# mihaidusmanu/local-feature-refinement

Measured on AMD Instinct MI355X. Metric: edges_per_s, higher is better.
Workload: dtype f64; 1 GPU; config4: synthetic match graph, 1344 images, 147000 tracks/GPU (mean length 6), 5001070 directed edges/GPU, Gaussian flows, seed 2+rank; edges_per_gpu=5001070, tracks_per_gpu=147000, components_per_gpu=147000, parallelism=components sharded, 1 rank(s), no data-path collective

## Files before the change

local-feature-refinement_amd/csrc/lfr_batch.hip:

```cpp
#include <hip/hip_runtime.h>

#include <algorithm>
#include <atomic>
#include <array>
#include <chrono>
#include <memory>
#include <string>
#include <thread>
#include <cstdio>
#include <cstdlib>
#include <cstring>
#include <vector>

#include "lfr_assemble.hpp"
#include "lfr_batch.hpp"
#include "lfr_internal.hpp"

using lfr::CompDesc;
using lfr::CompInfoDev;
using lfr::EdgeRec;
using lfr::KernelArgs;
using lfr::PackedRanges;
using lfr::block_lds_bytes;
using lfr::ensure_mirrors;
// ... 502 lines not shown
    return LFR_OK;
}

int lfr_hip_trim(int device) {
    lfr::DevCtx *ctx = lfr::dev_ctx(device);
    if (!ctx) return LFR_ERR_HIP;
    ctx->trim();
    return LFR_OK;
}

void lfr_batch_free(lfr_batch *b) { delete b; }

int lfr_batch_create(const lfr_problem *ph, int device, int shard_rank, int shard_world, int tukey_variant,
                     lfr_batch **out) {
    if (!ph || !out || shard_world < 1 || shard_rank < 0 || shard_rank >= shard_world ||
        (tukey_variant != LFR_TUKEY_CERES1 && tukey_variant != LFR_TUKEY_CERES2)) {
        lfr::set_error("bad argument"); return LFR_ERR_ARG;
    }
    *out = nullptr;
    const lfr::Problem &p = ph->p;
    lfr::DevCtx *ctx = lfr::dev_ctx(device);
    if (!ctx) return LFR_ERR_HIP;
    HIP_TRY(hipSetDevice(device));
    std::unique_ptr<lfr_batch> b(new lfr_batch());
    b->device = device; b->ctx = ctx; b->tukey_variant = tukey_variant; b->shard_world = shard_world;
    { const char *e = getenv("LFR_SERIAL_CLASSES"); b->serial = e && e[0] == '1'; }
    b->n_graph_nodes = p.g->n_nodes();
    b->graph = p.g; b->n_graph_matches = p.g->n_matches();
    int rc = p.host_batch ? create_from_host(b.get(), p, shard_rank, shard_world) : create_on_device(b.get(), p, shard_rank, shard_world);
    if (rc != LFR_OK) return rc;
    if ((rc = finish_workspace(b.get(), p)) != LFR_OK) return rc;
    host_trace("lfr_batch_create: workspace done");
    if (!(b->ev_fork = ctx->event_acquire(false))) return LFR_ERR_HIP;
    if (b->class_begin[lfr::KC_COUNT] > b->class_begin[lfr::KC_BLOCK]) {
        if (!(b->side_stream = ctx->side_stream(0))) return LFR_ERR_HIP;
        for (int cls = lfr::KC_BLOCK; cls < lfr::KC_COUNT; ++cls)
            if (b->class_begin[cls + 1] > b->class_begin[cls] && !(b->wg_stream[cls] = ctx->side_stream(1 + cls))) return LFR_ERR_HIP;
        {
            const int wg_begin = b->class_begin[lfr::KC_BLOCK], n_wg = b->class_begin[lfr::KC_COUNT] - wg_begin;
            hipStream_t so = ctx->s_main;
            size_t tmp_bytes = 0;
            HIP_TRY(rocprim::radix_sort_pairs<LfrRadixSortConfig>(nullptr, tmp_bytes, (const uint32_t *)nullptr, (uint32_t *)nullptr, (const uint32_t *)nullptr,
                                                                   (uint32_t *)nullptr, (size_t)n_wg, 0u, 27u, so));
            if (!b->order_slab.init(ctx, 16 * (size_t)n_wg + tmp_bytes + 4096)) return LFR_ERR_NOMEM;
            b->d_wg_order = b->order_slab.take_n<uint32_t>(n_wg);
            uint32_t *keys = b->order_slab.take_n<uint32_t>(n_wg), *keys_sorted = b->order_slab.take_n<uint32_t>(n_wg), *vals = b->order_slab.take_n<uint32_t>(n_wg);
            void *tmp = b->order_slab.take(tmp_bytes);
            if (!b->d_wg_order || !keys || !keys_sorted || !vals || !tmp) { lfr::set_error("order slab exhausted"); return LFR_ERR_NOMEM; }
            hipLaunchKernelGGL(k_wg_order_keys, dim3((n_wg + 255) / 256), dim3(256), 0, so, b->d_descs + wg_begin, n_wg,
                               b->class_begin[lfr::KC_BLOCK_M] - wg_begin, b->class_begin[lfr::KC_BLOCK_L] - wg_begin, b->class_begin[lfr::KC_GLOBAL] - wg_begin,
                               keys, vals, wg_begin);
            HIP_TRY(hipGetLastError());
            HIP_TRY(rocprim::radix_sort_pairs<LfrRadixSortConfig>(tmp, tmp_bytes, keys, keys_sorted, vals, b->d_wg_order, (size_t)n_wg, 0u, 27u, so));
            if (!(b->ev_order = ctx->event_acquire(false))) return LFR_ERR_HIP;
            HIP_TRY(hipEventRecord(b->ev_order, so));
        }
        host_trace("lfr_batch_create: hand-out order enqueued");
        const int lds_s = (int)block_lds_bytes(std::max(b->class_max_rows[lfr::KC_BLOCK], 2));
        const int lds_m = (int)block_lds_bytes(std::max(b->class_max_rows[lfr::KC_BLOCK_M], 2));
        const int lds_l = (int)block_lds_bytes(std::max(b->class_max_rows[lfr::KC_BLOCK_L], 2));
        if ((rc = lfr::reserve_block_lds(lds_s, lds_m, lds_l)) != LFR_OK) return rc;
    }
    {
        int64_t best = -1;
        for (int cls = 0; cls < lfr::KC_BLOCK; ++cls) if (b->class_edges[cls] > best) { best = b->class_edges[cls]; b->packed_slot = cls; }
    }
// ... 74 lines not shown
        HIP_TRY(hipGetLastError());
        return LFR_OK;
    };
    const bool have_side = b->class_begin[lfr::KC_COUNT] > b->class_begin[lfr::KC_BLOCK];
    if (b->serial) {
        for (int cls = 0; cls < lfr::KC_COUNT; ++cls) {
            a.desc_begin = b->class_begin[cls]; a.desc_end = b->class_begin[cls + 1]; a.cls = cls;
            const int n = a.desc_end - a.desc_begin;
            if (n <= 0) continue;
            recorded |= 1u << cls;
            HIP_TRY(hipEventRecord(b->ev[2 + 2 * cls], st));
            {
                const int grid = (n + kCompsPerBlock[cls] - 1) / kCompsPerBlock[cls];
                if (cls < lfr::KC_BLOCK) lfr::launch_group_class(cls, a, b->fused, grid, st);
                else { const int rc = launch_block(cls, st); if (rc != LFR_OK) return rc; }
                HIP_TRY(hipGetLastError());
            }
            HIP_TRY(hipEventRecord(b->ev[3 + 2 * cls], st));
        }
    } else {
        PackedRanges r;
        int nb = 0;
        for (int i = 0; i < 5; ++i) {
            const int cls = kPackedOrder[i];
            r.blk_begin[i] = nb;
            r.desc_begin[i] = b->class_begin[cls]; r.desc_end[i] = b->class_begin[cls + 1];
            const int n = r.desc_end[i] - r.desc_begin[i];
            nb += (n + kCompsPerBlock[cls] - 1) / kCompsPerBlock[cls];
        }
        r.blk_begin[5] = nb;
        const bool alias = !have_side && !materialised;
        auto launch_packed = [&](hipStream_t cs) -> int {
            if (!alias) HIP_TRY(hipEventRecord(b->ev[2 + 2 * b->packed_slot], cs));
            lfr::launch_packed(a, r, b->fused, nb, cs);
            HIP_TRY(hipGetLastError());
            if (!alias) HIP_TRY(hipEventRecord(b->ev[3 + 2 * b->packed_slot], cs));
            recorded |= 1u << b->packed_slot;
            if (alias) recorded |= kPackedEventsAliased;
            return LFR_OK;
        };
        auto launch_big = [&](int cls, hipStream_t cs) -> int {
            HIP_TRY(hipEventRecord(b->ev[2 + 2 * cls], cs));
            const int rc = launch_block(cls, cs);
            if (rc != LFR_OK) return rc;
            HIP_TRY(hipEventRecord(b->ev[3 + 2 * cls], cs));
            recorded |= 1u << cls;
            return LFR_OK;
        };
        if (!have_side) {
            if (nb > 0) { const int rc = launch_packed(st); if (rc != LFR_OK) return rc; }
        } else {
            static const std::array<int, 4> kBigOrder = [] {
                std::array<int, 4> o = {lfr::KC_GLOBAL, lfr::KC_BLOCK_M, lfr::KC_BLOCK_L, lfr::KC_BLOCK};
                if (const char *e = getenv("LFR_WG_ORDER")) {
                    int v[4];
                    if (sscanf(e, "%d,%d,%d,%d", &v[0], &v[1], &v[2], &v[3]) == 4) {
                        unsigned seen = 0;
                        for (int i = 0; i < 4; ++i) if (v[i] >= lfr::KC_BLOCK && v[i] < lfr::KC_COUNT) seen |= 1u << v[i];
                        if (seen == (0xfu << lfr::KC_BLOCK)) for (int i = 0; i < 4; ++i) o[i] = v[i];
                    }
                }
                return o;
            }();
            int first = -1, n_big = 0;
            for (int i = 0; i < 4; ++i) if (b->class_begin[kBigOrder[i] + 1] > b->class_begin[kBigOrder[i]]) { if (first < 0) first = kBigOrder[i]; ++n_big; }
            if (n_big > 1 || nb > 0) HIP_TRY(hipEventRecord(b->ev_fork, st));
            { const int rc = launch_big(first, st); if (rc != LFR_OK) return rc; }
            for (int i = 0; i < 4; ++i) {
// ... 470 lines not shown
```

local-feature-refinement_amd/csrc/lfr_batch.hpp:

```cpp
#pragma once

#include <hip/hip_runtime.h>

#include <cstdint>
#include <memory>
#include <vector>

#include "lfr_internal.hpp"

#define HIP_TRY(expr)                                                                         \
    do {                                                                                      \
        hipError_t _e = (expr);                                                               \
        if (_e != hipSuccess) {                                                               \
            lfr::set_error("%s failed: %s", #expr, hipGetErrorString(_e));                    \
            return LFR_ERR_HIP;                                                               \
        }                                                                                     \
    } while (0)

namespace lfr {

struct CompInfoDev {
    int32_t iterations, termination, n_successful, n_ls_evals, n_cand_evals, exec_passes;
    double final_cost;
};
// ... 82 lines not shown
    unsigned int *d_team_ctl = nullptr;
    double *d_team_red = nullptr;
    uint32_t team_work[3] = {0xffffffffu, 0xffffffffu, 0xffffffffu};
    int team_wgs = 0;
    uint32_t team_patience_us = 50000u;
    std::vector<int64_t> tree_comp_stats;
    int64_t tree_tiles = 0, tree_dense_tiles = 0;
    uint64_t *d_ws_off = nullptr, *d_es_off = nullptr;
    bool fused = false;
    uint32_t packed_edges = 0;
    uint32_t *d_edge_ref = nullptr, *d_edge_word = nullptr;
    std::shared_ptr<lfr::DevProblem> dev_hold;
    unsigned long long *d_prof = nullptr;
    lfr::NodeInc *d_node_inc = nullptr;
    uint32_t *d_in_idx = nullptr;
    uint32_t *d_desc_component = nullptr, *d_desc_class = nullptr, *d_desc_tracks = nullptr;
    bool mirrors_valid = false;
    std::vector<lfr::CompDesc> descs;
    std::vector<int64_t> desc_component;
    std::vector<int32_t> desc_class, desc_tracks;
    std::vector<uint32_t> node_ids;
    double *h_positions = nullptr;
    size_t h_positions_bytes = 0;
    float *h_positions_f32 = nullptr, *d_positions_f32 = nullptr;
    size_t h_positions_f32_bytes = 0, d_positions_f32_bytes = 0;
    static constexpr int kSlots = 64;
    static constexpr int kEvPerSlot = 2 * (lfr::KC_COUNT + 1);
    hipEvent_t ev_ring[kSlots * kEvPerSlot];
    hipEvent_t *ev = ev_ring;
    uint32_t ev_recorded[kSlots] = {};
    int64_t n_solves = 0;
    bool serial = false;
    hipEvent_t ev_fork = nullptr;
    lfr::DevArena order_slab;
    uint32_t *d_wg_order = nullptr;
    hipEvent_t ev_order = nullptr;
    hipStream_t side_stream = nullptr;
    hipStream_t wg_stream[lfr::KC_COUNT] = {nullptr};
    hipStream_t last_stream = nullptr;
    int packed_slot = 0;
    double h2d_ms = 0.0;
    std::vector<lfr::CompInfoDev> infos;
    bool infos_valid = false;
    const lfr::Graph *graph = nullptr;
    int64_t n_graph_matches = 0;
    BwdState *bwd = nullptr;
    CovState *cov = nullptr;

    lfr_batch() { for (auto &e : ev_ring) e = nullptr; }
    ~lfr_batch() {
        bwd_free(bwd);
        cov_free(cov);
        if (ctx) {
            (void)hipSetDevice(device);
            if (n_solves > 0) (void)hipStreamSynchronize(last_stream);
            if (side_stream) (void)hipStreamSynchronize(side_stream);
            for (auto &w : wg_stream) if (w) (void)hipStreamSynchronize(w);
            (void)hipStreamSynchronize(ctx->s_main);
            if (h_positions) ctx->pinned_release(h_positions, h_positions_bytes);
            if (h_positions_f32) ctx->pinned_release(h_positions_f32, h_positions_f32_bytes);
            if (d_positions_f32) ctx->dev_release(d_positions_f32, d_positions_f32_bytes);
        }
        if (ctx) {
            for (auto &e : ev_ring) ctx->event_release(e, true);
            ctx->event_release(ev_fork, false);
            ctx->event_release(ev_order, false);
        } else {
            for (auto &e : ev_ring) if (e) (void)hipEventDestroy(e);
        }
    }
};

namespace lfr {
int ensure_mirrors(lfr_batch *b);
void materialize_records(lfr_batch *b, hipStream_t st);
}
```

local-feature-refinement_amd/csrc/lfr_solve.hip:

```cpp
#include <hip/hip_runtime.h>

#include <algorithm>
#include <type_traits>
#include <cstdio>
#include <cstdlib>
#include <cstring>
#include <vector>

#include "lfr_batch.hpp"
#include "lfr_device.hpp"
#include "lfr_internal.hpp"

using namespace lfrdev;
using lfr::CompDesc;
using lfr::CompInfoDev;
using lfr::EdgeRec;
using lfr::KernelArgs;
using lfr::PackedRanges;
using lfr::block_lds_bytes;

namespace {

#ifdef LFR_PROFILE_PHASES
#define PROF_DECL unsigned long long pt_[7] = {0, 0, 0, 0, 0, 0, 0}; unsigned long long pt0_ = __builtin_amdgcn_s_memtime();
// ... 115 lines not shown
    };
    const int c_hi = (nv2_max + LPR - 1) / LPR;
#ifdef LFR_ABL_GJ
#define LFR_CL(n) do { lm_solve(std::integral_constant<int, n>{}); asm volatile("" : "+v"(rhs), "+v"(piv_own), "+v"(minpiv)); rhs = rhs0; piv_own = 1.0; minpiv = 1.0; lm_solve(std::integral_constant<int, n>{}); } while (0)
#else
#define LFR_CL(n) lm_solve(std::integral_constant<int, n>{})
#endif
    if constexpr (CPL == 8 && LPR == 1) {
        if (c_hi <= 2) LFR_CL(2); else if (c_hi <= 4) LFR_CL(4); else if (c_hi <= 6) LFR_CL(6); else LFR_CL(8);
    } else if constexpr (CPL == 8) {
        if (c_hi <= 4) LFR_CL(4); else if (c_hi <= 6) LFR_CL(6); else if (c_hi <= 7) LFR_CL(7); else LFR_CL(8);
    } else if constexpr (CPL == 32) {
        if (c_hi <= 18) LFR_CL(18); else if (c_hi <= 20) LFR_CL(20); else if (c_hi <= 22) LFR_CL(22);
        else LFR_CL(24);
    } else if constexpr (LPR == 1) {
        if (c_hi <= 10) LFR_CL(10); else if (c_hi <= 12) LFR_CL(12); else if (c_hi <= 14) LFR_CL(14); else LFR_CL(16);
    } else {
        if (c_hi <= 10) LFR_CL(10); else if (c_hi <= 12) LFR_CL(12); else if (c_hi <= 14) LFR_CL(14); else LFR_CL(16);
    }
#undef LFR_CL
    ISA_MARK("step_reductions");
    fail = !(minpiv > 0.0);
    return is_row ? -(rhs * fast_rcp(piv_own)) : 0.0;
}

#ifndef LFR_GROUP_WAVES
#define LFR_GROUP_WAVES 2
#endif
#ifndef LFR_PACKED_WAVES
#define LFR_PACKED_WAVES 1
#endif
constexpr int kPackedWaves = LFR_PACKED_WAVES;

template <int NV, int LPR, int EPL, bool FUSED>
__device__ __forceinline__ void solve_group_body(const KernelArgs &a, const int block_in_class, unsigned char *lds_raw) {
    constexpr int S = NV * LPR, G = 64 / S, CPL = NV / LPR, LD = NV + 1;
    static_assert(S <= 64 && (LPR == 1 || LPR == 2), "group geometry");
#ifdef LFR_ISA_MARKS
    asm volatile("; LFR_CLASS %0 %1 %2" :: "n"(NV), "n"(LPR), "n"(EPL));
#endif
    const int lane = threadIdx.x & 63, wave = threadIdx.x >> 6;
    const int gid = lane / S, sl = lane % S;
    const int row = sl % NV, part = sl / NV;
    const int ci0 = a.desc_begin + (block_in_class * kPackedWaves + wave) * G;
    if (ci0 >= a.desc_end) return;
#if defined(LFR_PROFILE_WGTIME) && LFR_PROFILE_WGTIME == 3
    const unsigned long long wave_r0_ = wall_clock64();
#endif
    const int ci = ci0 + gid;
    const bool have = ci < a.desc_end;
    GroupLds<NV> &L = reinterpret_cast<GroupLds<NV> *>(lds_raw)[wave * G + gid];

    CompDesc d;
    d.edge_off = 0; d.n_edges = 0; d.node_off = 0; d.n_nodes = 0; d.n_var = 0;
    if (have) d = a.descs[ci];
    const int n_var = d.n_var, nv2 = 2 * n_var, E = (int)d.n_edges;
    const int tv = a.tukey_variant;
    const bool is_row = row < nv2;
    const bool own = is_row && part == 0;
    int nv2_max = nv2;
#pragma unroll
    for (int m = 32; m >= 1; m >>= 1) nv2_max = max(nv2_max, __shfl_xor(nv2_max, m, 64));
    nv2_max = __builtin_amdgcn_readfirstlane(nv2_max);

#ifndef LFR_RES4
#define LFR_RES4 2
#endif
#ifndef LFR_RES16
#define LFR_RES16 3
#endif
    constexpr int RES = EPL <= 3 ? EPL : (NV == 16 ? LFR_RES16 : LFR_RES4);
    float flow[RES][18];
    float sim[RES];
    uint32_t idx[RES];
#pragma unroll
    for (int k = 0; k < RES; ++k) {
        const int e = sl + S * k;
        const bool on = e < E;
        load_packed_edge<FUSED>(a, d.edge_off + (on ? e : 0), flow[k], sim[k], idx[k]);
        if (!on) {
#pragma unroll
            for (int i = 0; i < 18; ++i) flow[k][i] = 0.f;
            sim[k] = 0.f; idx[k] = 0u;
        }
    }
    if (sl < NV) L.x[sl] = 0.0;
    if (sl < 2) L.x[NV + sl] = 0.0;
    for (int i = sl; i < NV * LD; i += S) L.A[i] = 0.0;

    int phase = have ? PH_EVAL_INIT : PH_DONE;
    double xi = 0.0, gi = 0.0, scale = 1.0, diag = 1.0;
    double inv_scale = 1.0;
    double xt = 0.0, delta = 0.0;
    double cost = 0.0, radius = kInitialRadius, x_norm = 0.0, gmax = 0.0;
    double g_dot_delta = 0.0, model_cost_change = 0.0, alpha = 1.0;
    int n_reject = 0;
    bool reuse_diagonal = false, step_successful = true, a_dirty = false;
    bool cost_only = false;
    int n_invalid = 0, iteration = 0, term = LFR_TERM_CONVERGENCE;
    if (sl == 0) { L.n_successful = 0; L.n_ls_evals = 0; L.n_cand = 0; L.exec_passes = 0; L.ls_iter = 0; L.ls_prev_flags = 0; }

    bool at_zero = true;
    constexpr bool kLogRegs = NV <= 16 && LPR == 1;
    LogCoef logc;
    if constexpr (kLogRegs) logc.load();
    const LogCoef *lcp = kLogRegs ? &logc : nullptr;
    PROF_DECL
    PROF_MARK(0);
    for (;;) {
        ISA_MARK("loop_top");
        if (!__any(phase != PH_DONE)) break;

        if (__any(phase == PH_SOLVE)) {
            bool ps = phase == PH_SOLVE;
            if (ps) {
                if (iteration >= kMaxIterations) { term = LFR_TERM_NO_CONVERGENCE; phase = PH_DONE; ps = false; }
                else if ((step_successful && gmax <= kGradientTol) || radius <= kMinRadius) { phase = PH_DONE; ps = false; }
                else if (a_dirty) { phase = PH_REEVAL; ps = false; if (own) L.x[row] = xi; }
            }
            if (__any(ps)) {
                wave_lds_sync();
                if (ps) { ++iteration; step_successful = false; }
                const double *A = L.A;
                const double aii = is_row ? A[row * LD + row] : 1.0;
                if (ps && !reuse_diagonal) diag = fmin(fmax(scale * scale * aii, kMinLmDiag), kMaxLmDiag);
                const double dd = diag * fast_rcp(radius) * (inv_scale * inv_scale);
                const double rhs0 = is_row ? gi : 0.0;
                bool fail = false;
                const double step = packed_step<NV, LPR>(A, row, part, is_row, nv2, nv2_max, dd, rhs0, fail, [&] { PROF_MARK(5); });
                const unsigned long long badmask = __ballot(is_row && !isfinite(step));
                const unsigned long long gmask = (S == 64) ? ~0ull : ((1ull << (S & 63)) - 1);
                const bool bad = ((badmask >> ((gid * S) & 63)) & gmask) != 0;
                const double dl = step;
                const double xt_full = clampb(__dadd_rn(xi, dl));
                double mcc = own ? (-rhs0 * step + dd * step * step) : 0.0, gdd = own ? gi * dl : 0.0;
                double sn2 = own ? (xi - xt_full) * (xi - xt_full) : 0.0, xn2 = own ? xt_full * xt_full : 0.0;
#ifdef LFR_ABL_RED
                { double a_ = mcc, b_ = gdd, c_ = sn2, d_ = xn2; asm volatile("" : "+v"(a_), "+v"(b_), "+v"(c_), "+v"(d_)); group_sum4<S>(a_, b_, c_, d_);
                  asm volatile("" :: "v"(a_), "v"(b_), "v"(c_), "v"(d_)); }
#endif
                group_sum4<S>(mcc, gdd, sn2, xn2);
                mcc *= 0.5;
                if (ps) {
                    reuse_diagonal = true;
                    const bool valid = !fail && !bad && mcc > 0.0;
                    if (!valid) {
                        if (++n_invalid >= kMaxInvalid) { term = LFR_TERM_FAILURE; phase = PH_DONE; }
                        else { radius = ldexp(radius, -(1 + n_reject)); ++n_reject; }
                    } else {
                        n_invalid = 0;
                        model_cost_change = mcc; delta = dl; g_dot_delta = gdd;
                        alpha = 1.0;
                        cost_only = mcc <= kFunctionTol * cost;
                        if (sl == 0) { L.step_norm2 = sn2; L.xnorm2 = xn2; L.ls_iter = 0; L.ls_prev_flags = 0; }
                        xt = xt_full;
                        if (own) L.x[row] = xt;
                        phase = PH_EVAL_LS;
                    }
                }
            }
        }

        PROF_MARK(1);
        const bool pe = phase == PH_EVAL_INIT || phase == PH_EVAL_LS || phase == PH_EVAL_CAND || phase == PH_REEVAL;
        if (!__any(pe)) continue;
        const bool jac = !cost_only;
        if (pe && jac) {
            double2 *A2 = reinterpret_cast<double2 *>(L.A);
            for (int i = sl; i < (nv2 * LD + 1) / 2; i += S) A2[i] = make_double2(0.0, 0.0);
            if (sl < NV / 2) reinterpret_cast<double2 *>(L.g)[sl] = make_double2(0.0, 0.0);
#ifdef LFR_ABL_ZERO
            wave_lds_sync();
            for (int i = sl; i < (nv2 * LD + 1) / 2; i += S) A2[i] = make_double2(0.0, 0.0);
#endif
        }
        wave_lds_sync();
        PROF_MARK(6);
        double cost_l = 0.0;
        if (__any(pe && jac)) {
            ISA_MARK("sweep_setup");
#pragma unroll
            for (int k = 0; k < EPL; ++k) {
                if (!(pe && sl + S * k < E)) continue;
                float flow_k[18]; float sim_k; uint32_t pk;
                if (k < RES) {
#pragma unroll
                    for (int i = 0; i < 18; ++i) flow_k[i] = flow[k < RES ? k : 0][i];
                    sim_k = sim[k < RES ? k : 0]; pk = idx[k < RES ? k : 0];
                } else {
                    load_packed_edge<FUSED>(a, d.edge_off + (sl + S * k), flow_k, sim_k, pk);
                }
                asm volatile("" : "+v"(pk));
                const int es = (int)(pk & 0xffffu), ed = (int)((pk >> 16) & 0x7fffu), ekind = (int)(pk >> 31);
                const int xa = 2 * min(es, n_var), xb = 2 * min(ed, n_var);
                const int ra = es < n_var ? 2 * es : -1, rb = ed < n_var ? 2 * ed : -1;
                EdgeOut o;
                ISA_MARK("eval");
                eval_edge<true>(flow_k, sim_k, ekind, tv, L.x[xa], L.x[xa + 1], L.x[xb], L.x[xb + 1], o, at_zero, lcp);
#ifdef LFR_ABL_EVAL
// ... 32 lines not shown
                }
            }
        } else {
#pragma unroll
            for (int k = 0; k < EPL; ++k) {
                if (!(pe && sl + S * k < E)) continue;
                float flow_k[18]; float sim_k; uint32_t pk;
                if (k < RES) {
#pragma unroll
                    for (int i = 0; i < 18; ++i) flow_k[i] = flow[k < RES ? k : 0][i];
                    sim_k = sim[k < RES ? k : 0]; pk = idx[k < RES ? k : 0];
                } else {
                    load_packed_edge<FUSED>(a, d.edge_off + (sl + S * k), flow_k, sim_k, pk);
                }
                asm volatile("" : "+v"(pk));
                const int es = (int)(pk & 0xffffu), ed = (int)((pk >> 16) & 0x7fffu), ekind = (int)(pk >> 31);
                const int xa = 2 * min(es, n_var), xb = 2 * min(ed, n_var);
                const int ra = es < n_var ? 2 * es : -1, rb = ed < n_var ? 2 * ed : -1;
                EdgeOut o;
                (void)ra; (void)rb;
                ISA_MARK("eval_cost_only");
                eval_edge<false>(flow_k, sim_k, ekind, tv, L.x[xa], L.x[xa + 1], L.x[xb], L.x[xb + 1], o, false, lcp);
                ISA_MARK("cost_only_loop");
                cost_l += o.cost;
            }
        }
        at_zero = false;
        wave_lds_sync();
        PROF_MARK(2);
#ifdef LFR_ABL_RED
        { double a_ = cost_l; asm volatile("" : "+v"(a_)); a_ = group_sum<S>(a_); asm volatile("" :: "v"(a_)); a_ = group_max<S>(a_); asm volatile("" :: "v"(a_)); }
#endif
        const double cost_e = group_sum<S>(cost_l);
        const double xe = (phase == PH_EVAL_INIT || phase == PH_REEVAL) ? xi : xt;
        const double gnew = is_row ? L.g[row] : 0.0;
        const double gmax_new = group_max<S>(is_row ? fabs(xe - clampb(xe - gnew)) : 0.0);
        const double step_norm2 = L.step_norm2, xnorm2_new = L.xnorm2;

        PROF_MARK(3);
        bool decide = false;
        double cost_cand = 0.0;
        if (pe && sl == 0) atomicAdd(&L.exec_passes, 1);
        if (phase == PH_EVAL_INIT) {
            cost = cost_e; gi = gnew; gmax = gmax_new;
            inv_scale = is_row ? 1.0 + sqrt(L.A[row * LD + row]) : 1.0;
            scale = 1.0 / inv_scale;
            a_dirty = false; phase = PH_SOLVE;
        } else if (phase == PH_REEVAL) {
            a_dirty = false; phase = PH_SOLVE;
        } else if (phase == PH_EVAL_LS && cost_only) {
            cost_only = false;
            const bool armijo = isfinite(cost_e) && !(cost_e > cost + kLsSufficientDecrease * g_dot_delta * alpha);
            const double ptol = kParameterTol * (x_norm + kParameterTol);
            const bool stop = armijo && (step_norm2 <= ptol * ptol || fabs(cost - cost_e) <= kFunctionTol * cost);
            if (stop) {
                if (sl == 0) atomicAdd(&L.n_ls_evals, 1);
                decide = true; cost_cand = cost_e;
            }
        } else if (phase == PH_EVAL_LS) {
            if (sl == 0) atomicAdd(&L.n_ls_evals, 1);
            const bool value_valid = isfinite(cost_e);
            if (value_valid && !(cost_e > cost + kLsSufficientDecrease * g_dot_delta * alpha)) {
                decide = true; cost_cand = cost_e;
            } else {
                const double gdc = group_sum<S>(own ? delta * gnew : 0.0);
                const double dir_max = group_max<S>(fabs(delta));
// ... 24 lines not shown
                if (sl == 0) { L.step_norm2 = sn2; L.xnorm2 = xn2; }
            }
        } else if (phase == PH_EVAL_CAND) {
            decide = true; cost_cand = isfinite(cost_e) ? cost_e : DBL_MAX;
        }
        if (decide) {
            if (sl == 0) atomicAdd(&L.n_cand, 1);
            const double cost_change = cost - cost_cand;
            const double ptol = kParameterTol * (x_norm + kParameterTol);
            if (step_norm2 <= ptol * ptol) phase = PH_DONE;
            else if (fabs(cost_change) <= kFunctionTol * cost) phase = PH_DONE;
            else {
                const double rel = cost_change * fast_rcp(model_cost_change);
                if (rel > kMinRelDecrease) {
                    xi = xt; x_norm = fast_sqrt(xnorm2_new); cost = cost_cand; gi = gnew; gmax = gmax_new;
                    step_successful = true;
                    if (sl == 0) atomicAdd(&L.n_successful, 1);
                    const double t = 2.0 * rel - 1.0;
                    radius = fmin(kMaxRadius, radius * fast_rcp(fmax(1.0 / 3.0, 1.0 - t * t * t)));
                    n_reject = 0; reuse_diagonal = false; a_dirty = false;
                } else {
                    radius = ldexp(radius, -(1 + n_reject)); ++n_reject;
                    a_dirty = true;
                }
                phase = PH_SOLVE;
            }
        }
        PROF_MARK(4);
    }
    PROF_FLUSH();

    if (have) {
        if (own)
            a.positions[2 * (size_t)a.node_ids[d.node_off + (row >> 1)] + (row & 1)] = term != LFR_TERM_FAILURE ? xi : 0.0;
        if (sl == 0) {
            CompInfoDev inf;
            inf.iterations = iteration; inf.termination = term; inf.n_successful = L.n_successful;
            inf.n_ls_evals = L.n_ls_evals; inf.n_cand_evals = L.n_cand; inf.exec_passes = L.exec_passes;
            inf.final_cost = cost;
#if defined(LFR_PROFILE_WGTIME) && LFR_PROFILE_WGTIME == 3
            inf.final_cost = (double)wave_r0_;
            inf.n_ls_evals = inf.iterations;
            inf.iterations = (int)(wall_clock64() - wave_r0_);
            const unsigned hw = __builtin_amdgcn_s_getreg((4 << 0) | (0 << 6) | (31 << 11));
            const unsigned xcc = __builtin_amdgcn_s_getreg((20 << 0) | (0 << 6) | (3 << 11));
            inf.termination = (int)((hw & 0xffffu) | ((xcc & 0xfu) << 16));
#endif
            a.infos[ci] = inf;
        }
    }
}

constexpr size_t kPackedLdsBytes = kPackedWaves * (sizeof(GroupLds<16>) * 4 > 2 * sizeof(GroupLds<32>) ? sizeof(GroupLds<16>) * 4 : 2 * sizeof(GroupLds<32>));
static_assert(kPackedLdsBytes >= kPackedWaves * 8 * sizeof(GroupLds<8>) && kPackedLdsBytes >= kPackedWaves * 2 * sizeof(GroupLds<16>), "LDS budget");

template <int NV, int LPR, int EPL, bool FUSED>
__global__ __launch_bounds__(64 * kPackedWaves, LFR_GROUP_WAVES) void solve_group_kernel(const KernelArgs a) {
    __shared__ __attribute__((aligned(16))) unsigned char lds_raw[kPackedWaves * (64 / (NV * LPR)) * sizeof(GroupLds<NV>)];
    solve_group_body<NV, LPR, EPL, FUSED>(a, (int)blockIdx.x, lds_raw);
}

template <bool FUSED>
__global__ __launch_bounds__(64 * kPackedWaves, LFR_GROUP_WAVES) void solve_packed_kernel(KernelArgs a, const PackedRanges r) {
    __shared__ __attribute__((aligned(16))) unsigned char lds_raw[kPackedLdsBytes];
    const int b = (int)blockIdx.x;
    if (b < r.blk_begin[1]) {
        a.desc_begin = r.desc_begin[0]; a.desc_end = r.desc_end[0]; a.cls = lfr::KC_G64_4;
        solve_group_body<32, 2, 5, FUSED>(a, b - r.blk_begin[0], lds_raw);
    } else if (b < r.blk_begin[2]) {
        a.desc_begin = r.desc_begin[1]; a.desc_end = r.desc_end[1]; a.cls = lfr::KC_G64_2;
        solve_group_body<32, 1, 6, FUSED>(a, b - r.blk_begin[1], lds_raw);
    } else if (b < r.blk_begin[3]) {
        a.desc_begin = r.desc_begin[2]; a.desc_end = r.desc_end[2]; a.cls = lfr::KC_G32;
    } else if (b < r.blk_begin[4]) {
        a.desc_begin = r.desc_begin[3]; a.desc_end = r.desc_end[3]; a.cls = lfr::KC_G16;
        solve_group_body<16, 1, 6, FUSED>(a, b - r.blk_begin[3], lds_raw);
    } else {
        a.desc_begin = r.desc_begin[4]; a.desc_end = r.desc_end[4]; a.cls = lfr::KC_G8;
        solve_group_body<8, 1, 3, FUSED>(a, b - r.blk_begin[4], lds_raw);
    }
}


__device__ __forceinline__ void mat_add(double *p, double v) { __hip_atomic_fetch_add(p, v, __ATOMIC_RELAXED, __HIP_MEMORY_SCOPE_WORKGROUP); }
__device__ __forceinline__ uint32_t tri(int i, int j) { return (__umul24((unsigned)i, (unsigned)i + 1u) >> 1) + (unsigned)j; }

struct BlockShared {
    double red[16];
    double bcast[4];
    int flag;
    int ready;
    int lead;
    int lead_t;
    int wbar;
    int ovf;
};

using f64x4 = __attribute__((ext_vector_type(4))) double;

__device__ __forceinline__ double uni(double v) {
    return __hiloint2double(__builtin_amdgcn_readfirstlane(__double2hiint(v)), __builtin_amdgcn_readfirstlane(__double2loint(v)));
}

struct LmSearch {
    LsSample initial, previous, current;
    __device__ __forceinline__ void set_gradient(double g) { current.gradient = g; current.gradient_valid = isfinite(g); }
};

struct LmControl {
    enum Verdict { STOP, ACCEPT, REJECT };
    double cost, gmax, x_norm = 0.0, radius = kInitialRadius, decrease_factor = 2.0;
    bool reuse_diagonal = false, step_successful = true, matrix_valid = true;
// ... 2125 lines not shown
__global__ void lfr_warmup_kernel(int *p) { if (p) *p = 0; }

}

namespace lfr {

const SolveGeometry &solve_geometry() {
    static const SolveGeometry g = {kPackedWaves, {8 * kPackedWaves, 4 * kPackedWaves, 2 * kPackedWaves, 2 * kPackedWaves, kPackedWaves, 1, 1, 1, 1},
                                    kThreadsS, kThreadsM, kThreadsL, kThreadsG, kTeamMax, kTeamUnitsPerXcc, kTeamCtlWords, kTeamRedPerUnit};
    return g;
}

size_t block_lds_bytes(int max_rows) {
    return (block_vector_doubles(max_rows) - (size_t)max_rows + (size_t)(max_rows + 1) * (max_rows + 2) / 2) * sizeof(double);
}

int reserve_block_lds(int lds_s, int lds_m, int lds_l) {
    HIP_TRY(hipFuncSetAttribute((const void *)solve_block_kernel<kThreadsS>, hipFuncAttributeMaxDynamicSharedMemorySize, lds_s));
    HIP_TRY(hipFuncSetAttribute((const void *)solve_block_kernel<kThreadsM>, hipFuncAttributeMaxDynamicSharedMemorySize, std::max(lds_m, kThreadsM == kThreadsS ? lds_s : 0)));
    HIP_TRY(hipFuncSetAttribute((const void *)solve_block_kernel<kThreadsL>, hipFuncAttributeMaxDynamicSharedMemorySize,
                                std::max(lds_l, std::max(kThreadsL == kThreadsM ? lds_m : 0, kThreadsL == kThreadsS ? lds_s : 0))));
    return LFR_OK;
}

void launch_packed(const KernelArgs &a, const PackedRanges &r, bool fused, int n_blocks, hipStream_t cs) {
    const dim3 blk(64 * kPackedWaves);
    if (fused) hipLaunchKernelGGL(solve_packed_kernel<true>, dim3(n_blocks), blk, 0, cs, a, r);
    else hipLaunchKernelGGL(solve_packed_kernel<false>, dim3(n_blocks), blk, 0, cs, a, r);
}

void launch_group_class(int cls, const KernelArgs &a, bool fused, int n_blocks, hipStream_t st) {
    const dim3 grid(n_blocks), blk(64 * kPackedWaves);
    switch (cls) {
        case lfr::KC_G8:    if (fused) hipLaunchKernelGGL((solve_group_kernel<8, 1, 3, true>), grid, blk, 0, st, a); else hipLaunchKernelGGL((solve_group_kernel<8, 1, 3, false>), grid, blk, 0, st, a); break;
        case lfr::KC_G16:   if (fused) hipLaunchKernelGGL((solve_group_kernel<16, 1, 6, true>), grid, blk, 0, st, a); else hipLaunchKernelGGL((solve_group_kernel<16, 1, 6, false>), grid, blk, 0, st, a); break;
        case lfr::KC_G32:   break;
        case lfr::KC_G64_2: if (fused) hipLaunchKernelGGL((solve_group_kernel<32, 1, 6, true>), grid, blk, 0, st, a); else hipLaunchKernelGGL((solve_group_kernel<32, 1, 6, false>), grid, blk, 0, st, a); break;
        case lfr::KC_G64_4: if (fused) hipLaunchKernelGGL((solve_group_kernel<32, 2, 5, true>), grid, blk, 0, st, a); else hipLaunchKernelGGL((solve_group_kernel<32, 2, 5, false>), grid, blk, 0, st, a); break;
    }
}

void launch_block_class(int cls, const KernelArgs &a, int rows, int wgs, hipStream_t cs) {
    const size_t lds = block_lds_bytes(rows);
    switch (cls) {
        case lfr::KC_BLOCK:   hipLaunchKernelGGL((solve_block_kernel<kThreadsS>), dim3(wgs), dim3(kThreadsS), lds, cs, a, rows); break;
        case lfr::KC_BLOCK_M: hipLaunchKernelGGL((solve_block_kernel<kThreadsM>), dim3(wgs), dim3(kThreadsM), lds, cs, a, rows); break;
        case lfr::KC_BLOCK_L: hipLaunchKernelGGL((solve_block_kernel<kThreadsL>), dim3(wgs), dim3(kThreadsL), lds, cs, a, rows); break;
    }
}

void launch_tree(const KernelArgs &a, bool team, int grid, hipStream_t cs) {
    if (team) hipLaunchKernelGGL((solve_tree_team_kernel<kThreadsG>), dim3(grid), dim3(kThreadsG), 0, cs, a);
    else hipLaunchKernelGGL((solve_tree_kernel<kThreadsG>), dim3(grid), dim3(kThreadsG), 0, cs, a);
}

void launch_warmup() { hipLaunchKernelGGL(lfr_warmup_kernel, dim3(1), dim3(64), 0, nullptr, (int *)nullptr); }

}

extern "C" {

namespace {
__global__ void eval_edges_kernel(int64_t n, const float *flows, const float *sim, const int32_t *kind, const double *x1,
                                  const double *x2, int tukey_variant, double *out8, double *cost_only) {
    const int64_t i = (int64_t)blockIdx.x * blockDim.x + threadIdx.x;
    if (i >= n) return;
    float fl[18];
    for (int k = 0; k < 18; ++k) fl[k] = flows[18 * i + k];
// ... 287 lines not shown
```

Baseline: 12.45 billion edges/s.

## Split small group classes into register-diet kernels on forked side streams

Removes the G16 and G8 classes from the packed kernel and launches them as separate group kernels on side streams, with fork and join events around the remaining packed launch. The new 'diet' variant parks per-row and uniform solver scalars in LDS across the Gauss-Jordan step and the residual evaluation. It also shrinks the residual register caches and drops register-resident log coefficients, so the kernels can run with a higher waves-per-EU launch bound. The intent is to raise occupancy for the many small components and overlap them with the larger classes. The cost is extra LDS traffic, more synchronisation and more launch and event overhead.

```diff
diff --git a/local-feature-refinement_amd/csrc/lfr_batch.hip b/local-feature-refinement_amd/csrc/lfr_batch.hip
--- a/local-feature-refinement_amd/csrc/lfr_batch.hip
+++ b/local-feature-refinement_amd/csrc/lfr_batch.hip
@@ -558,6 +558,12 @@
     if ((rc = finish_workspace(b.get(), p)) != LFR_OK) return rc;
     host_trace("lfr_batch_create: workspace done");
     if (!(b->ev_fork = ctx->event_acquire(false))) return LFR_ERR_HIP;
+    if (!b->serial) {
+        if (!(b->ev_small_fork = ctx->event_acquire(false))) return LFR_ERR_HIP;
+        for (int i = 0; i < 2; ++i) if (!(b->ev_small_join[i] = ctx->event_acquire(false))) return LFR_ERR_HIP;
+        for (int cls : {lfr::KC_G16, lfr::KC_G8})
+            if (b->class_begin[cls + 1] > b->class_begin[cls] && !(b->wg_stream[cls] = ctx->side_stream(1 + cls))) return LFR_ERR_HIP;
+    }
     if (b->class_begin[lfr::KC_COUNT] > b->class_begin[lfr::KC_BLOCK]) {
         if (!(b->side_stream = ctx->side_stream(0))) return LFR_ERR_HIP;
         for (int cls = lfr::KC_BLOCK; cls < lfr::KC_COUNT; ++cls)
@@ -698,8 +704,28 @@
         const bool alias = !have_side && !materialised;
         auto launch_packed = [&](hipStream_t cs) -> int {
             if (!alias) HIP_TRY(hipEventRecord(b->ev[2 + 2 * b->packed_slot], cs));
-            lfr::launch_packed(a, r, b->fused, nb, cs);
-            HIP_TRY(hipGetLastError());
+            const int nb32 = r.blk_begin[3];
+            const int small_cls[2] = {lfr::KC_G16, lfr::KC_G8};
+            int small_nb[2] = {r.blk_begin[4] - r.blk_begin[3], r.blk_begin[5] - r.blk_begin[4]};
+            bool on_cs = false, forked = false;
+            if (nb32 > 0) { lfr::launch_packed(a, r, b->fused, nb32, cs); HIP_TRY(hipGetLastError()); on_cs = true; }
+            hipStream_t joined[2] = {nullptr, nullptr};
+            for (int i = 0; i < 2; ++i) {
+                if (small_nb[i] <= 0) continue;
+                KernelArgs as = a;
+                as.desc_begin = r.desc_begin[3 + i]; as.desc_end = r.desc_end[3 + i]; as.cls = small_cls[i];
+                hipStream_t ss = cs;
+                if (on_cs) {
+                    ss = b->wg_stream[small_cls[i]];
+                    if (!forked) { HIP_TRY(hipEventRecord(b->ev_small_fork, cs)); forked = true; }
+                    HIP_TRY(hipStreamWaitEvent(ss, b->ev_small_fork, 0));
+                }
+                lfr::launch_group_class(small_cls[i], as, b->fused, small_nb[i], ss);
+                HIP_TRY(hipGetLastError());
+                if (ss != cs) { HIP_TRY(hipEventRecord(b->ev_small_join[i], ss)); joined[i] = ss; }
+                on_cs = true;
+            }
+            for (int i = 0; i < 2; ++i) if (joined[i]) HIP_TRY(hipStreamWaitEvent(cs, b->ev_small_join[i], 0));
             if (!alias) HIP_TRY(hipEventRecord(b->ev[3 + 2 * b->packed_slot], cs));
             recorded |= 1u << b->packed_slot;
             if (alias) recorded |= kPackedEventsAliased;
diff --git a/local-feature-refinement_amd/csrc/lfr_batch.hpp b/local-feature-refinement_amd/csrc/lfr_batch.hpp
--- a/local-feature-refinement_amd/csrc/lfr_batch.hpp
+++ b/local-feature-refinement_amd/csrc/lfr_batch.hpp
@@ -138,6 +138,7 @@
     int64_t n_solves = 0;
     bool serial = false;
     hipEvent_t ev_fork = nullptr;
+    hipEvent_t ev_small_fork = nullptr, ev_small_join[2] = {nullptr, nullptr};
     lfr::DevArena order_slab;
     uint32_t *d_wg_order = nullptr;
     hipEvent_t ev_order = nullptr;
@@ -170,6 +171,8 @@
         if (ctx) {
             for (auto &e : ev_ring) ctx->event_release(e, true);
             ctx->event_release(ev_fork, false);
+            ctx->event_release(ev_small_fork, false);
+            for (auto &e : ev_small_join) ctx->event_release(e, false);
             ctx->event_release(ev_order, false);
         } else {
             for (auto &e : ev_ring) if (e) (void)hipEventDestroy(e);
diff --git a/local-feature-refinement_amd/csrc/lfr_solve.hip b/local-feature-refinement_amd/csrc/lfr_solve.hip
--- a/local-feature-refinement_amd/csrc/lfr_solve.hip
+++ b/local-feature-refinement_amd/csrc/lfr_solve.hip
@@ -171,10 +171,27 @@
 #endif
 constexpr int kPackedWaves = LFR_PACKED_WAVES;
 
-template <int NV, int LPR, int EPL, bool FUSED>
+#ifndef LFR_PARK_ROW
+#define LFR_PARK_ROW 5
+#endif
+#ifndef LFR_PARK_UNI
+#define LFR_PARK_UNI 6
+#endif
+template <int NV>
+struct alignas(16) GroupLdsDiet : GroupLds<NV> {
+    static constexpr int kRow = NV == 8 ? 7 : LFR_PARK_ROW, kUni = NV == 8 ? 7 : LFR_PARK_UNI;
+    double park_row[kRow > 0 ? kRow : 1][NV];
+    double park_uni[kUni > 0 ? kUni + (kUni & 1) : 2];
+};
+
+__device__ __forceinline__ int park_lane(int sl) { asm volatile("" : "+v"(sl)); return sl; }
+
+template <int NV, int LPR, int EPL, bool FUSED, bool DIET = false>
 __device__ __forceinline__ void solve_group_body(const KernelArgs &a, const int block_in_class, unsigned char *lds_raw) {
     constexpr int S = NV * LPR, G = 64 / S, CPL = NV / LPR, LD = NV + 1;
     static_assert(S <= 64 && (LPR == 1 || LPR == 2), "group geometry");
+    static_assert(!DIET || LPR == 1, "the parked row state is one cell per lane");
+    using LdsT = std::conditional_t<DIET, GroupLdsDiet<NV>, GroupLds<NV>>;
 #ifdef LFR_ISA_MARKS
     asm volatile("; LFR_CLASS %0 %1 %2" :: "n"(NV), "n"(LPR), "n"(EPL));
 #endif
@@ -188,7 +205,7 @@
 #endif
     const int ci = ci0 + gid;
     const bool have = ci < a.desc_end;
-    GroupLds<NV> &L = reinterpret_cast<GroupLds<NV> *>(lds_raw)[wave * G + gid];
+    LdsT &L = reinterpret_cast<LdsT *>(lds_raw)[wave * G + gid];
 
     CompDesc d;
     d.edge_off = 0; d.n_edges = 0; d.node_off = 0; d.n_nodes = 0; d.n_var = 0;
@@ -208,7 +225,16 @@
 #ifndef LFR_RES16
 #define LFR_RES16 3
 #endif
-    constexpr int RES = EPL <= 3 ? EPL : (NV == 16 ? LFR_RES16 : LFR_RES4);
+#ifndef LFR_DIET_RES8
+#define LFR_DIET_RES8 1
+#endif
+#ifndef LFR_DIET_RES16
+#define LFR_DIET_RES16 1
+#endif
+#ifndef LFR_DIET_LOGREGS
+#define LFR_DIET_LOGREGS 0
+#endif
+    constexpr int RES = DIET ? (NV == 16 ? LFR_DIET_RES16 : (EPL < LFR_DIET_RES8 ? EPL : LFR_DIET_RES8)) : EPL <= 3 ? EPL : (NV == 16 ? LFR_RES16 : LFR_RES4);
     float flow[RES][18];
     float sim[RES];
     uint32_t idx[RES];
@@ -240,7 +266,7 @@
     if (sl == 0) { L.n_successful = 0; L.n_ls_evals = 0; L.n_cand = 0; L.exec_passes = 0; L.ls_iter = 0; L.ls_prev_flags = 0; }
 
     bool at_zero = true;
-    constexpr bool kLogRegs = NV <= 16 && LPR == 1;
+    constexpr bool kLogRegs = NV <= 16 && LPR == 1 && (!DIET || LFR_DIET_LOGREGS);
     LogCoef logc;
     if constexpr (kLogRegs) logc.load();
     const LogCoef *lcp = kLogRegs ? &logc : nullptr;
@@ -266,7 +292,27 @@
                 const double dd = diag * fast_rcp(radius) * (inv_scale * inv_scale);
                 const double rhs0 = is_row ? gi : 0.0;
                 bool fail = false;
+#ifndef LFR_DIET_PARK_GJ
+#define LFR_DIET_PARK_GJ 1
+#endif
+                if constexpr (DIET && LFR_DIET_PARK_GJ) {
+                    double *const rv[5] = {&scale, &inv_scale, &diag, &delta, &xt};
+                    double *const uv[6] = {&model_cost_change, &g_dot_delta, &alpha, &x_norm, &gmax, &cost};
+#pragma unroll
+                    for (int i = 0; i < (LdsT::kRow < 5 ? LdsT::kRow : 5); ++i) { L.park_row[i][park_lane(sl)] = *rv[i]; asm volatile("" : "=v"(*rv[i])); }
+#pragma unroll
+                    for (int i = 0; i < (LdsT::kUni < 6 ? LdsT::kUni : 6); ++i) { if (sl == 0) L.park_uni[i] = *uv[i]; asm volatile("" : "=v"(*uv[i])); }
+                }
                 const double step = packed_step<NV, LPR>(A, row, part, is_row, nv2, nv2_max, dd, rhs0, fail, [&] { PROF_MARK(5); });
+                if constexpr (DIET && LFR_DIET_PARK_GJ) {
+                    double *const rv[5] = {&scale, &inv_scale, &diag, &delta, &xt};
+                    double *const uv[6] = {&model_cost_change, &g_dot_delta, &alpha, &x_norm, &gmax, &cost};
+                    wave_lds_sync();
+#pragma unroll
+                    for (int i = 0; i < (LdsT::kRow < 5 ? LdsT::kRow : 5); ++i) *rv[i] = L.park_row[i][park_lane(sl)];
+#pragma unroll
+                    for (int i = 0; i < (LdsT::kUni < 6 ? LdsT::kUni : 6); ++i) *uv[i] = L.park_uni[i];
+                }
                 const unsigned long long badmask = __ballot(is_row && !isfinite(step));
                 const unsigned long long gmask = (S == 64) ? ~0ull : ((1ull << (S & 63)) - 1);
                 const bool bad = ((badmask >> ((gid * S) & 63)) & gmask) != 0;
@@ -304,6 +350,14 @@
         const bool pe = phase == PH_EVAL_INIT || phase == PH_EVAL_LS || phase == PH_EVAL_CAND || phase == PH_REEVAL;
         if (!__any(pe)) continue;
         const bool jac = !cost_only;
+        if constexpr (DIET) {
+            double *const rv[7] = {&scale, &inv_scale, &diag, &delta, &gi, &xt, &xi};
+            double *const uv[7] = {&model_cost_change, &g_dot_delta, &alpha, &x_norm, &gmax, &radius, &cost};
+#pragma unroll
+            for (int i = 0; i < LdsT::kRow; ++i) { L.park_row[i][park_lane(sl)] = *rv[i]; asm volatile("" : "=v"(*rv[i])); }
+#pragma unroll
+            for (int i = 0; i < LdsT::kUni; ++i) { if (sl == 0) L.park_uni[i] = *uv[i]; asm volatile("" : "=v"(*uv[i])); }
+        }
         if (pe && jac) {
             double2 *A2 = reinterpret_cast<double2 *>(L.A);
             for (int i = sl; i < (nv2 * LD + 1) / 2; i += S) A2[i] = make_double2(0.0, 0.0);
@@ -402,6 +456,14 @@
         { double a_ = cost_l; asm volatile("" : "+v"(a_)); a_ = group_sum<S>(a_); asm volatile("" :: "v"(a_)); a_ = group_max<S>(a_); asm volatile("" :: "v"(a_)); }
 #endif
         const double cost_e = group_sum<S>(cost_l);
+        if constexpr (DIET) {
+            double *const rv[7] = {&scale, &inv_scale, &diag, &delta, &gi, &xt, &xi};
+            double *const uv[7] = {&model_cost_change, &g_dot_delta, &alpha, &x_norm, &gmax, &radius, &cost};
+#pragma unroll
+            for (int i = 0; i < LdsT::kRow; ++i) *rv[i] = L.park_row[i][park_lane(sl)];
+#pragma unroll
+            for (int i = 0; i < LdsT::kUni; ++i) *uv[i] = L.park_uni[i];
+        }
         const double xe = (phase == PH_EVAL_INIT || phase == PH_REEVAL) ? xi : xt;
         const double gnew = is_row ? L.g[row] : 0.0;
         const double gmax_new = group_max<S>(is_row ? fabs(xe - clampb(xe - gnew)) : 0.0);
@@ -492,7 +554,7 @@
 
     if (have) {
         if (own)
-            a.positions[2 * (size_t)a.node_ids[d.node_off + (row >> 1)] + (row & 1)] = term != LFR_TERM_FAILURE ? xi : 0.0;
+            a.positions[2 * (size_t)a.node_ids[(DIET ? a.descs[ci].node_off : d.node_off) + (row >> 1)] + (row & 1)] = term != LFR_TERM_FAILURE ? xi : 0.0;
         if (sl == 0) {
             CompInfoDev inf;
             inf.iterations = iteration; inf.termination = term; inf.n_successful = L.n_successful;
@@ -514,11 +576,16 @@
 constexpr size_t kPackedLdsBytes = kPackedWaves * (sizeof(GroupLds<16>) * 4 > 2 * sizeof(GroupLds<32>) ? sizeof(GroupLds<16>) * 4 : 2 * sizeof(GroupLds<32>));
 static_assert(kPackedLdsBytes >= kPackedWaves * 8 * sizeof(GroupLds<8>) && kPackedLdsBytes >= kPackedWaves * 2 * sizeof(GroupLds<16>), "LDS budget");
 
-template <int NV, int LPR, int EPL, bool FUSED>
-__global__ __launch_bounds__(64 * kPackedWaves, LFR_GROUP_WAVES) void solve_group_kernel(const KernelArgs a) {
-    __shared__ __attribute__((aligned(16))) unsigned char lds_raw[kPackedWaves * (64 / (NV * LPR)) * sizeof(GroupLds<NV>)];
-    solve_group_body<NV, LPR, EPL, FUSED>(a, (int)blockIdx.x, lds_raw);
-}
+constexpr int kSmallWaves = 3;
+constexpr size_t kSmallLdsBytes = kPackedWaves * (8 * sizeof(GroupLdsDiet<8>) > 4 * sizeof(GroupLdsDiet<16>) ? 8 * sizeof(GroupLdsDiet<8>) : 4 * sizeof(GroupLdsDiet<16>));
+static_assert(4 * kSmallWaves * kSmallLdsBytes <= 163840 * kPackedWaves, "twelve waves of the small classes must fit the CU's 160 KB of LDS");
+
+template <int NV, int LPR, int EPL, bool FUSED, bool DIET = false>
+__global__ __launch_bounds__(64 * kPackedWaves, DIET ? kSmallWaves : LFR_GROUP_WAVES) void solve_group_kernel(const KernelArgs a) {
+    __shared__ __attribute__((aligned(16))) unsigned char lds_raw[kPackedWaves * (64 / (NV * LPR)) * sizeof(std::conditional_t<DIET, GroupLdsDiet<NV>, GroupLds<NV>>)];
+    solve_group_body<NV, LPR, EPL, FUSED, DIET>(a, (int)blockIdx.x, lds_raw);
+}
+
 
 template <bool FUSED>
 __global__ __launch_bounds__(64 * kPackedWaves, LFR_GROUP_WAVES) void solve_packed_kernel(KernelArgs a, const PackedRanges r) {
@@ -530,14 +597,6 @@
     } else if (b < r.blk_begin[2]) {
         a.desc_begin = r.desc_begin[1]; a.desc_end = r.desc_end[1]; a.cls = lfr::KC_G64_2;
         solve_group_body<32, 1, 6, FUSED>(a, b - r.blk_begin[1], lds_raw);
-    } else if (b < r.blk_begin[3]) {
-        a.desc_begin = r.desc_begin[2]; a.desc_end = r.desc_end[2]; a.cls = lfr::KC_G32;
-    } else if (b < r.blk_begin[4]) {
-        a.desc_begin = r.desc_begin[3]; a.desc_end = r.desc_end[3]; a.cls = lfr::KC_G16;
-        solve_group_body<16, 1, 6, FUSED>(a, b - r.blk_begin[3], lds_raw);
-    } else {
-        a.desc_begin = r.desc_begin[4]; a.desc_end = r.desc_end[4]; a.cls = lfr::KC_G8;
-        solve_group_body<8, 1, 3, FUSED>(a, b - r.blk_begin[4], lds_raw);
     }
 }
 
@@ -2729,8 +2788,8 @@
 void launch_group_class(int cls, const KernelArgs &a, bool fused, int n_blocks, hipStream_t st) {
     const dim3 grid(n_blocks), blk(64 * kPackedWaves);
     switch (cls) {
-        case lfr::KC_G8:    if (fused) hipLaunchKernelGGL((solve_group_kernel<8, 1, 3, true>), grid, blk, 0, st, a); else hipLaunchKernelGGL((solve_group_kernel<8, 1, 3, false>), grid, blk, 0, st, a); break;
-        case lfr::KC_G16:   if (fused) hipLaunchKernelGGL((solve_group_kernel<16, 1, 6, true>), grid, blk, 0, st, a); else hipLaunchKernelGGL((solve_group_kernel<16, 1, 6, false>), grid, blk, 0, st, a); break;
+        case lfr::KC_G8:    if (fused) hipLaunchKernelGGL((solve_group_kernel<8, 1, 3, true, true>), grid, blk, 0, st, a); else hipLaunchKernelGGL((solve_group_kernel<8, 1, 3, false, true>), grid, blk, 0, st, a); break;
+        case lfr::KC_G16:   if (fused) hipLaunchKernelGGL((solve_group_kernel<16, 1, 6, true, true>), grid, blk, 0, st, a); else hipLaunchKernelGGL((solve_group_kernel<16, 1, 6, false, true>), grid, blk, 0, st, a); break;
         case lfr::KC_G32:   break;
         case lfr::KC_G64_2: if (fused) hipLaunchKernelGGL((solve_group_kernel<32, 1, 6, true>), grid, blk, 0, st, a); else hipLaunchKernelGGL((solve_group_kernel<32, 1, 6, false>), grid, blk, 0, st, a); break;
         case lfr::KC_G64_4: if (fused) hipLaunchKernelGGL((solve_group_kernel<32, 2, 5, true>), grid, blk, 0, st, a); else hipLaunchKernelGGL((solve_group_kernel<32, 2, 5, false>), grid, blk, 0, st, a); break;
```

Result: slower. 10.82 billion edges/s (-13.1%).
